# ZhonghuaYi/FocusFlow_official

Measured on AMD Instinct MI355X. Metric: frame-pairs/sec FF-RAFT 384x512 iters=12, higher is better.
Workload: dtype f32 via fp16x3 split operands on the f16 MFMA pipe (f32 accumulate, fp32-level accuracy); 1 GPU; FF-RAFT forward (test_mode), 8 pairs/GPU 384x512, iters=12, fp32 correlation pyramid, random-init weights, ORB-like masks (BASELINE configs[1]); pairs_per_gpu=8, corr_pyramid=fp32, conv_precision=f16x3, hipgraph=False, skip_unused_upsample=False, parallelism=dp1 (independent shards, no collective)

## Files before the change

### focusflow_official_amd/_hip.py

```python
import ctypes as C
import os

_PKG = os.path.dirname(os.path.abspath(__file__))
LIB_PATH = os.path.join(_PKG, "lib", "libfocusflow_hip.so")
if os.environ.get("FF_LAB_LIB"):
    LIB_PATH = os.path.join(_PKG, "lib", os.environ["FF_LAB_LIB"])

ACT_NONE, ACT_RELU, ACT_SIGMOID, ACT_TANH, ACT_LEAKY = 0, 1, 2, 3, 4
W_F32, W_F16X3, W_F16 = 0, 1, 2
MAX_SEG = 3
_fp = C.c_void_p
_ll = C.c_longlong


class FFFusionPair(C.Structure):
    _fields_ = [
        ("x", _fp * 2), ("x_ld", C.c_int * 2), ("xres", _fp * 2), ("xres_ld", C.c_int * 2), ("scale", _fp * 2), ("shift", _fp * 2),
        ("in_act", C.c_int), ("w_frag", _fp * 2), ("bias", _fp * 2), ("w_format", C.c_int), ("y", _fp * 2), ("y_ld", C.c_int * 2),
        ("B", C.c_int), ("HW", C.c_int), ("C", C.c_int),
    ]


class FFEncoderTail(C.Structure):
    _fields_ = [
        ("x", _fp * 2), ("x_ld", C.c_int * 2), ("xres", _fp * 2), ("xres_ld", C.c_int * 2), ("scale", _fp * 2), ("shift", _fp * 2),
        ("in_act", C.c_int), ("w_frag", _fp), ("bias", _fp), ("w_format", C.c_int), ("y", _fp), ("y_ld", C.c_int),
        ("B", C.c_int), ("HW", C.c_int), ("C", C.c_int), ("Cout", C.c_int),
    ]


class FFConvParams(C.Structure):
    _fields_ = [
        ("x", _fp * MAX_SEG), ("x_ld", C.c_int * MAX_SEG), ("x_c", C.c_int * MAX_SEG),
        ("x_gstride", _ll * MAX_SEG), ("groups", C.c_int), ("B", C.c_int), ("H", C.c_int), ("W", C.c_int),
        ("w", _fp), ("w_gstride", _ll), ("bias", _fp), ("ch_scale", _fp), ("ch_shift", _fp),
        ("out_scale", C.c_float), ("res", _fp), ("res_ld", C.c_int), ("y", _fp), ("y_ld", C.c_int),
        ("y_gstride", _ll), ("Ho", C.c_int), ("Wo", C.c_int), ("Cout", C.c_int),
        ("KH", C.c_int), ("KW", C.c_int), ("stride", C.c_int), ("pad_h", C.c_int), ("pad_w", C.c_int),
        ("act", C.c_int), ("act_res", C.c_int), ("w_format", C.c_int),
        ("dil_h", C.c_int), ("dil_w", C.c_int), ("x_amax", _fp),
        ("in_scale", _fp), ("in_shift", _fp), ("in_act", C.c_int),
        ("res2", _fp), ("res2_ld", C.c_int), ("res_split", C.c_int),
        ("splitk_ws", _fp), ("splitk", C.c_int),
        ("ep_mode", C.c_int), ("ep_split", C.c_int), ("ep_a", _fp), ("ep_a_ld", C.c_int), ("ep_b", _fp), ("ep_b_ld", C.c_int),
        ("stats_part", _fp),
        ("x_fmt", C.c_int * MAX_SEG), ("y_fmt", C.c_int), ("y_fmt_from", C.c_int), ("y2", _fp), ("y2_ld", C.c_int),
        ("w_frag", _fp),
    ]


PACK_MAX_MEMBERS = 4
PACK_MAX_SLICES = 4


class FFPackJob(C.Structure):
    _fields_ = [
        ("w", _fp * PACK_MAX_MEMBERS), ("bias", _fp * PACK_MAX_MEMBERS),
        ("cout_m", C.c_int * PACK_MAX_MEMBERS), ("off", C.c_int * PACK_MAX_MEMBERS), ("nmem", C.c_int), ("cout", C.c_int),
        ("cin_src", C.c_int), ("nslice", C.c_int), ("slice_lo", C.c_int * PACK_MAX_SLICES), ("slice_hi", C.c_int * PACK_MAX_SLICES),
        ("cin", C.c_int), ("cin_pad", C.c_int), ("KH", C.c_int), ("KW", C.c_int),
# ... 34 lines not shown
    "ff_corr_lookup_tiled_bwd_all": [_fp, C.POINTER(_fp), C.POINTER(_fp), C.c_int, C.c_int, _ll, C.c_int, C.c_int, _fp],
    "ff_corr_lookup_tiled_bwd": [C.POINTER(_fp), _fp, _fp, C.c_int, _ll, C.c_int, C.c_int, _fp],
    "ff_corr_pyramid_tiled_bwd": [_fp, _fp, _fp, _fp, _ll, C.c_int, C.c_int, _fp],
    "ff_corr_alt_prepare": [_fp, _fp, C.c_int, C.c_int, C.c_int, C.c_int, C.c_int, _fp, C.POINTER(_fp), _fp],
    "ff_corr_alt_lookup": [_fp, C.POINTER(_fp), C.c_int, _fp, C.c_int, C.c_int, C.c_int, _fp, C.c_int, _fp, _fp],
    "ff_corr_alt_lookup_bwd": [_fp, C.POINTER(_fp), C.POINTER(_fp), C.POINTER(_fp), C.c_int, C.c_int, C.c_int, C.c_int, C.c_int, _fp,
                               C.POINTER(_fp), _fp],
    "ff_act_copy": [_fp, C.c_int, _fp, C.c_int, _ll, C.c_int, C.c_int, _fp],
    "ff_range_probe": [_fp, C.c_int, _ll, C.c_int, _fp, _fp],
    "ff_split_copy": [_fp, C.c_int, _fp, C.c_int, _ll, C.c_int, C.c_int, C.c_int, _fp],
    "ff_coords_init": [_fp, _fp, C.c_int, C.c_int, C.c_int, _fp],
    "ff_forward_interpolate": [_fp, _fp, _fp, C.c_int, C.c_int, C.c_int, _fp],
    "ff_good_features": [_fp, C.c_int, _ll, _ll, _ll, C.c_int, C.c_int, C.c_int, C.c_int, C.c_double, C.c_int, _fp, _fp, _fp, _fp, _fp],
    "ff_frame_ingest": [_fp, _ll, _ll, _ll, _ll, C.c_int, C.c_int, C.c_int, C.c_int, C.c_int, C.c_int, C.c_int, C.c_int, _fp, _fp],
    "ff_pad_replicate": [_fp, C.c_int, _ll, _ll, _ll, C.c_int, C.c_int, C.c_int, C.c_int, C.c_int, C.c_int, C.c_int, _fp, _fp],
    "ff_keypoint_matches": [_fp, _fp, C.c_int, _fp, _ll, _ll, _ll, _ll, C.c_int, C.c_int, C.c_int, C.c_int, C.c_int, C.c_int, C.c_int, _fp, _fp, _fp],
    "ff_tracks_replenish": [_fp, _fp, _fp, _fp, C.c_int, _fp, _fp, C.c_int, C.c_int, C.c_int, C.c_int, C.c_int, _fp, _fp, _fp],
    "ff_tracks_mask": [_fp, _fp, C.c_int, C.c_int, C.c_int, C.c_int, _fp, _fp],
    "ff_tracks_advance": [_fp, _fp, _fp, C.c_int, _fp, _ll, _ll, _ll, _ll, C.c_int, C.c_int, C.c_int, C.c_int, C.c_int, C.c_int, C.c_int, _fp, _fp, _fp,
                          _fp, _fp],
    "ff_fb_dense": [_fp, _ll, _ll, _ll, _ll, _fp, _ll, _ll, _ll, _ll, C.c_int, C.c_int, C.c_int, C.c_int, C.c_int, C.c_int, C.c_int, C.c_float, C.c_float,
                    _fp, _fp, _fp],
    "ff_fb_matches": [_fp, _fp, C.c_int, _fp, _ll, _ll, _ll, _ll, C.c_int, C.c_int, C.c_int, C.c_int, C.c_int, C.c_int, C.c_int, C.c_float, C.c_float,
                      _fp, _fp, _fp, _fp, _fp, _fp],
    "ff_epipolar_ransac": [_fp, _fp, C.c_int, C.c_int, C.c_int, C.c_int, C.c_float, C.c_int, C.c_int, C.c_int, C.c_uint, _fp, C.c_int, _fp, _fp, _fp, _fp,
                           _fp, _fp, _fp, _fp, _fp, _fp, _ll, _fp],
    "ff_coords_step": [_fp, _fp, C.c_int, _fp, _fp, C.c_int, C.c_int, C.c_int, C.c_int, _fp],
    "ff_gru_pass": [C.c_int, _fp, C.c_int, _fp, C.c_int, _fp, C.c_int, _fp, C.c_int, _fp, C.c_int, _fp, _fp, _fp, _fp, C.c_int, _fp, C.c_int, _fp, C.c_int,
                    C.c_int, C.c_int, C.c_int, _fp],
    "ff_gru_pass_rec": [C.c_int, _fp, C.c_int, _fp, C.c_int, _fp, C.c_int, _fp, C.c_int, _fp, C.c_int, _fp, _fp, _fp, _fp, C.c_int, _fp, C.c_int, _fp, C.c_int,
                        _fp, _fp, _fp, C.c_int, C.c_int, C.c_int, C.c_int, _fp],
    "ff_fusion_pair_fwd": [C.POINTER(FFFusionPair), _fp],
    "ff_encoder_tail_fwd": [C.POINTER(FFEncoderTail), _fp],
    "ff_gru_rh": [_fp, C.c_int, _fp, C.c_int, _fp, C.c_int, _ll, C.c_int, _fp],
    "ff_gru_blend": [_fp, C.c_int, _fp, C.c_int, _fp, C.c_int, _fp, C.c_int, _ll, C.c_int, _fp],
    "ff_upsample_flow": [_fp, C.c_int, _fp, C.c_int, _fp, C.c_int, C.c_int, C.c_int, _fp],
    "ff_nhwc_to_nchw": [_fp, C.c_int, _fp, C.c_int, C.c_int, C.c_int, C.c_int, _fp],
    "ff_conv2d_wgrad": [C.POINTER(FFConvParams), _fp, _ll, _fp, _fp],
    "ff_unpack_conv_wgrad": [_fp, C.c_int, C.c_int, C.c_int, C.c_int, C.c_int, C.c_int, _fp, _fp],
    "ff_pack_conv_weight_dgrad": [_fp, C.c_int, C.c_int, C.c_int, C.c_int, _fp, C.c_int, C.c_int, _fp],
    "ff_act_bwd": [_fp, C.c_int, _fp, C.c_int, _fp, C.c_int, _ll, C.c_int, C.c_int, C.c_int, C.c_float, _fp, _fp],
    "ff_deconv4x4s2_small": [_fp, C.c_int, C.c_int, C.c_int, C.c_int, C.c_int, _fp, _fp, C.c_int, _fp, C.c_int, _fp],
    "ff_dilate2": [_fp, C.c_int, _fp, C.c_int, C.c_int, C.c_int, C.c_int, C.c_int, C.c_int, _fp],
    "ff_norm_bwd": [_fp, C.c_int, _fp, C.c_int, _fp, C.c_int, _fp, _fp, C.c_int, C.c_int, C.c_float, _fp, _fp,
                    C.c_int, _fp, C.c_int, _fp, C.c_int, C.c_int, C.c_int, C.c_int, _fp, _fp],
    "ff_gru_rh_bwd": [_fp, C.c_int, _fp, C.c_int, _fp, C.c_int, _fp, C.c_int, _fp, C.c_int, _ll, C.c_int, _fp],
    "ff_gru_blend_bwd": [_fp, C.c_int, _fp, C.c_int, _fp, C.c_int, _fp, C.c_int, _fp, C.c_int, _fp, C.c_int,
                         _fp, C.c_int, _ll, C.c_int, _fp],
    "ff_upsample_flow_bwd": [_fp, _fp, C.c_int, _fp, C.c_int, _fp, _fp, C.c_int, C.c_int, C.c_int, _fp],
    "ff_upsample_flow_bwd_ex": [_fp, _fp, C.c_int, _fp, C.c_int, _fp, C.c_int, _fp, C.c_float, _fp, C.c_int, C.c_int, C.c_int, _fp],
    "ff_gru_bwd_blend": [_fp, C.c_int, _fp, C.c_int, _fp, C.c_int, _fp, C.c_int, _fp, C.c_int, _fp, C.c_int, _fp, C.c_int, _fp, C.c_int, _fp, C.c_int,
                         _fp, _fp, _ll, C.c_int, _fp],
    "ff_gru_bwd_rh": [_fp, C.c_int, _fp, C.c_int, _fp, C.c_int, _fp, C.c_int, _fp, C.c_int, _fp, C.c_int, C.c_int, _fp, _ll, C.c_int, _fp],
    "ff_gru_bwd_out": [_fp, C.c_int, _fp, C.c_int, _fp, C.c_int, _fp, C.c_int, _fp, C.c_int, _fp, C.c_int, C.c_int, _fp, _ll, C.c_int, _fp],
    "ff_sum_stack": [_fp, C.c_int, _ll, _fp, _fp],
    "ff_pwc_costvolume_fwd": [_fp, C.c_int, _fp, C.c_int, _fp, C.c_int, C.c_int, C.c_int, C.c_int, C.c_int, _fp],
    "ff_pwc_costvolume_fwd_ex": [_fp, C.c_int, _fp, C.c_int, _fp, C.c_int, C.c_int, C.c_int, C.c_int, C.c_int, C.c_int, _fp, C.c_int, _fp],
    "ff_pwc_costvolume_bwd": [_fp, C.c_int, _fp, C.c_int, _fp, C.c_int, C.c_int, C.c_int, C.c_int, C.c_int, _fp],
    "ff_pwc_gout_transpose": [_fp, C.c_int, _fp, C.c_int, C.c_int, C.c_int, C.c_int, _fp],
    "ff_pwc_backwarp": [_fp, C.c_int, _fp, C.c_int, C.c_float, _fp, C.c_int, C.c_int, C.c_int, C.c_int, C.c_int, _fp],
    "ff_loss_prepare": [_fp, _fp, _fp, _fp, C.c_int, C.c_float, _fp, _fp, _fp, C.c_int, C.c_int, C.c_int, _fp],
    "ff_loss_accumulate": [_fp, _fp, _fp, _fp, _fp, C.c_float, C.c_float, C.c_float, _fp, _fp, C.c_int, C.c_int,
                           C.c_int, _fp],
    "ff_epe_metric": [_fp, _fp, _fp, _fp, C.c_int, C.c_int, C.c_int, _fp],
    "ff_nchw_to_nhwc4": [_fp, C.c_int, C.c_float, _fp, C.c_int, C.c_int, C.c_int, _fp],
    "ff_resize_bilinear": [_fp, C.c_int, C.c_int, C.c_int, C.c_int, _fp, C.c_int, C.c_int, C.c_int, C.c_float, C.c_float, _fp],
    "ff_pwc_backwarp_bwd": [_fp, C.c_int, _fp, C.c_int, C.c_float, _fp, C.c_int, _fp, C.c_int, _fp, C.c_int, C.c_int, C.c_int, C.c_int,
                            C.c_int, _fp],
    "ff_pwc_loss_mask": [_fp, _fp, C.c_int, _fp, _fp, C.c_int, C.c_int, C.c_int, C.c_int, C.c_int, _fp],
    "ff_pwc_loss_scale": [_fp, _fp, _fp, _fp, C.c_float, C.c_float, C.c_int, C.c_int, C.c_int, C.c_float, C.c_float, _fp, _fp, C.c_int,
                          C.c_int, C.c_int, C.c_int, C.c_int, _fp],
    "ff_pwc_epe_mean": [_fp, _fp, C.c_int, C.c_float, C.c_float, _fp, C.c_int, C.c_int, C.c_int, _fp],
    "ff_pwc_loss_scale_sparse": [_fp, _fp, _fp, _fp, C.c_float, C.c_float, C.c_int, C.c_int, C.c_int, C.c_float, C.c_float, _fp, _fp, C.c_int,
                                 C.c_int, C.c_int, C.c_int, C.c_int, _fp],
    "ff_pwc_epe_mean_sparse": [_fp, _fp, C.c_int, C.c_float, C.c_float, _fp, C.c_int, C.c_int, C.c_int, _fp],
    "ff_resize_to_nhwc4": [_fp, C.c_int, C.c_int, C.c_int, _fp, C.c_int, C.c_int, C.c_int, _fp],
    "ff_png_unfilter": [_fp, _ll, C.c_int, C.c_int, C.c_int, _fp],
    "ff_mask_prepare": [C.c_int, _fp, _fp, _fp, C.c_int, _fp, _fp, _fp, C.c_int, C.c_int, C.c_int, _fp],
    "ff_chan_stats_fwd": [_fp, C.c_int, C.c_int, _ll, _fp, C.c_int, _fp, _fp],
    "ff_chan_stats_bwd": [_fp, C.c_int, _fp, C.c_int, _ll, _fp, C.c_int, _fp],
    "ff_spatial_stats_fwd": [_fp, C.c_int, C.c_int, C.c_int, C.c_int, _fp, _fp, _fp, _fp, _fp],
    "ff_spatial_stats_bwd": [_fp, _fp, _fp, C.c_int, C.c_int, C.c_int, _fp, C.c_int, _fp],
    "ff_scale_add_fwd": [_fp, C.c_int, _fp, C.c_int, _fp, _fp, C.c_int, _fp, C.c_int, C.c_int, C.c_int, C.c_int, C.c_int, _fp],
    "ff_scale_add_bwd": [_fp, C.c_int, _fp, C.c_int, _fp, C.c_int, _fp, _fp, C.c_int, _fp, _fp, C.c_int, C.c_int, C.c_int,
                         C.c_int, _fp],
}
EXPORTS = sorted(list(_SIGS) + ["ff_last_error", "ff_abi_version", "ff_corr_plane_elems", "ff_conv2d_splitk_hint", "ff_conv2d_stats_parts", "ff_fusion_pair_tile",
                                 "ff_forward_interpolate_ws", "ff_good_features_ws", "ff_epipolar_ws"])

ABI_VERSION = 7
_lib = None


class FocusFlowHipError(RuntimeError):
    pass


_ABLATION_VARS = ("FF_LOOKUP_ABLATE", "FF_LOOKUP_ABLATE3", "FF_CORR_BUILD_ABLATE", "FF_PATCH_ABLATE")
_TUNING_VARS = ("FF_DMA_TILE", "FF_GRU_PASS_TH", "FF_LAB_LIB")


def lab_variables_set():
    return [v for v in _ABLATION_VARS + _TUNING_VARS if os.environ.get(v) is not None]


def load():
    global _lib
    if _lib is not None:
        return _lib
    abl = [v for v in _ABLATION_VARS if os.environ.get(v) is not None]
    if abl and not os.environ.get("FF_LAB_LIB"):
        raise FocusFlowHipError(f"{', '.join(abl)} set in the environment: timing-only ablations return wrong results and are not part of "
                                "libfocusflow_hip.so; unset them (the lab build under tools/ is where they live)")
    if not os.path.exists(LIB_PATH):
        raise FocusFlowHipError(
            f"{LIB_PATH} is missing: build it with `python -m focusflow_official_amd.build` "
            "(hipcc --offload-arch=gfx950).  There is no CPU/PyTorch fallback for the hot path.")
    lib = C.CDLL(LIB_PATH)
    for name, argtypes in _SIGS.items():
        fn = getattr(lib, name, None)
        if fn is None:
            raise FocusFlowHipError(f"{LIB_PATH} does not export {name}: it was built from older sources; "
                                    "rebuild with `python -m focusflow_official_amd.build`")
        fn.argtypes = argtypes
        fn.restype = C.c_int
    lib.ff_last_error.restype = C.c_char_p
    lib.ff_last_error.argtypes = []
    lib.ff_abi_version.restype = C.c_int
    lib.ff_abi_version.argtypes = []
    lib.ff_corr_plane_elems.restype = C.c_int
    lib.ff_corr_plane_elems.argtypes = [C.c_int, C.c_int, C.c_int, C.c_int]
    lib.ff_conv2d_splitk_hint.restype = C.c_int
    lib.ff_conv2d_splitk_hint.argtypes = [C.POINTER(FFConvParams)]
    lib.ff_fusion_pair_tile.restype = C.c_int
    lib.ff_fusion_pair_tile.argtypes = [C.c_int]
    lib.ff_forward_interpolate_ws.restype = C.c_int
    lib.ff_forward_interpolate_ws.argtypes = [C.c_int, C.c_int, C.c_int]
    lib.ff_good_features_ws.restype = C.c_int
    lib.ff_good_features_ws.argtypes = [C.c_int, C.c_int, C.c_int]
    lib.ff_epipolar_ws.restype = C.c_int
    lib.ff_epipolar_ws.argtypes = [C.c_int, C.c_int, C.c_int]
    lib.ff_conv2d_stats_parts.restype = C.c_int
    lib.ff_conv2d_stats_parts.argtypes = [C.POINTER(FFConvParams)]
    got = lib.ff_abi_version()
    if got != ABI_VERSION:
        raise FocusFlowHipError(f"{LIB_PATH} speaks ABI version {got}, these bindings (FFConvParams layout, argument lists) "
                                f"version {ABI_VERSION}: rebuild with `python -m focusflow_official_amd.build`")
    _lib = lib
    return lib


def call(name, *args):
    lib = load()
    rc = getattr(lib, name)(*args)
    if rc != 0:
        raise FocusFlowHipError(f"{name} failed ({rc}): {lib.ff_last_error().decode()}")
```

### focusflow_official_amd/cce.py

```python
from typing import Tuple, Optional, Sequence

import ctypes
import os
import weakref

import torch
import torch.nn as nn

from . import _hip, fn, ops
from .ops import ACT_NONE, ACT_RELU, ACT_SIGMOID

EPS = 1e-5


_NORM_ON_LOAD = True


_ALL_PACKED = weakref.WeakSet()
_DMA_FRAG = True
_PREPACK = True
_serial = [0]


class PackedConv:
# ... 275 lines not shown
            blk += (J.items_fwd + J.items_dgrad + 255) // 256
            arr[i] = J
        host = torch.frombuffer(bytearray(bytes(arr)), dtype=torch.uint8)
        cache = owner.__dict__["_ff_pack_table"] = (sig, host.to(device), len(jobs), blk)
    ops.pack_weights_table(cache[1], cache[2], cache[3])
    for (pc, nf, nd, kf, kd), (J, fmt, dfmt) in zip(todo, jobs):
        if nf:
            pc.w, pc.fmt, pc._key = (pc._w_raw if fmt == 0 else pc._w_split), fmt, kf
            pc._gen += 1
        if nd:
            pc.wd, pc.dfmt, pc._dkey = (pc._wd_raw if dfmt == 0 else pc._wd_split), dfmt, kd
    return len(todo)


def train_streams() -> bool:
    v = os.environ.get("FF_TRAIN_STREAMS")
    if v is not None:
        return v != "0"
    return not (torch.distributed.is_available() and torch.distributed.is_initialized())
_BRANCH_STREAMS = True
_branch_streams = {}


def _branch_stream(device):
    key = (torch.device(device).index, torch.cuda.current_stream(device).cuda_stream)
    if key not in _branch_streams:
        _branch_streams[key] = torch.cuda.Stream(device=device)
    return _branch_streams[key]


_FUSION_PAIR = os.environ.get("FF_FUSION_PAIR", "1") != "0"
_PAIR_FUSION = True
_ENCODER_TAIL = True
_W_LIMIT = 4094.0


def invalidate_packed(module: nn.Module) -> int:
    ids = {id(p) for p in module.parameters()}
    n = 0
    for pc in list(_ALL_PACKED):
        if id(pc.convs[0]._parameters["weight"]) in ids:
            pc._key = pc._dkey = None
            n += 1
    for m in module.modules():
        if hasattr(m, "_ff_fold"):
            del m._ff_fold
            n += 1
        if getattr(m, "_pair_key", None) is not None:
            m._pair_key = None
            n += 1
        if getattr(m, "_tail_key", None) is not None:
            m._tail_key = None
            n += 1
        if getattr(m, "_mask2_stage_of", None) is not None:
            m._mask2_stage = m._mask2_stage_of = None
            n += 1
    return n


def _make_norm(kind: str, c: int):
    if kind == "batch":
        return nn.BatchNorm2d(c)
    if kind == "instance":
        return nn.InstanceNorm2d(c)
    if kind == "none":
        return nn.Sequential()
# ... 167 lines not shown
                    return ops.LazyAct(y, st, y.shape[1] * y.shape[2], EPS, act, res)
                return ops.norm_apply(y, st, True, EPS, act=act, res=res, out=y)
            if ops.CONV_STATS_TRAIN:
                y, st = fn.conv(pc, x, want_stats=True, take_res=take_res)
            else:
                y = fn.conv(pc, x, take_res=take_res)
                st = ops.norm_stats(y.detach(), per_sample=True)
            return fn.NormFn.apply(y, None, None, res, True, False, EPS, relu, st, defer_res)
        if self.norm_fn == "batch":
            if norm.training:
                y = fn.conv(pc, x, take_res=take_res and taped)
                st = ops.norm_stats(y.detach(), per_sample=False)
                b, h, w, _ = y.shape
                ops.bn_update_running(norm, st, b * h * w)
                norm.num_batches_tracked += 1
                if taped:
                    return fn.NormFn.apply(y, norm.weight, norm.bias, res, False, False, norm.eps, relu, st, defer_res)
                return ops.norm_apply(y, st, False, norm.eps, norm.weight, norm.bias, act=act, res=res, out=y)
            if taped:
                y = fn.conv(pc, x, take_res=take_res)
                n = float(y.shape[0] * y.shape[1] * y.shape[2])
                rm, rv = norm.running_mean.double(), norm.running_var.double()
                st = torch.stack([rm * n, (rv + rm * rm) * n], -1)[None].contiguous()
                return fn.NormFn.apply(y, norm.weight, norm.bias, res, False, True, norm.eps, relu, st, defer_res)
            sc, sh = ops.bn_fold(norm)
            return pc(x, act=act, ch_scale=sc, ch_shift=sh, res=res, act_res=ACT_RELU)
        if taped:
            raise NotImplementedError("norm_fn='none' has no autograd path (unused by the reference configs)")
        return pc(x, act=act, res=res, act_res=ACT_RELU)

    def _block_recorded(self, blk: ResidualBlock, x) -> bool:
        return torch.is_grad_enabled() and x.requires_grad and self.norm_fn in ("instance", "batch")

    def _block(self, blk: ResidualBlock, x, lazy_out=False):
        p2 = blk._p2
        if (_NORM_ON_LOAD and self.norm_fn == "instance" and not torch.is_grad_enabled() and ops.w_format() in (_hip.W_F16X3, _hip.W_F16)
                and p2.cin % 32 == 0 and (p2.kh, p2.kw, p2.stride) == (3, 3, 1)):
            t1, st = blk._p1(x, want_stats=True)
            sc, sh = ops.norm_coeffs(st, t1.shape[1] * t1.shape[2], EPS)
            if blk.downsample is not None:
                x = self._conv_norm(x, blk._pd, blk.norm3, ACT_NONE)
            t2, st2 = p2(t1, in_scale=sc, in_shift=sh, in_act=ACT_RELU, want_stats=True)
            if lazy_out:
                return ops.LazyAct(t2, st2, t2.shape[1] * t2.shape[2], EPS, ACT_RELU, x)
            return ops.norm_apply(t2, st2, True, EPS, act=ACT_RELU, res=x, out=t2)
        fuse = blk.downsample is None and self._block_recorded(blk, x) and fn.res_grad_fused(blk._p1)
        y = self._conv_norm(x, blk._p1, blk.norm1, ACT_RELU, take_res=fuse)
        if blk.downsample is not None:
            x = self._conv_norm(x, blk._pd, blk.norm3, ACT_NONE)
        return self._conv_norm(y, blk._p2, blk.norm2, ACT_RELU, res=x, lazy=lazy_out and self.norm_fn == "instance" and not torch.is_grad_enabled(),
                               defer_res=fuse)

    def _run_stage(self, stage, x, lazy_out=False):
        if lazy_out:
            return self._block(stage[1], self._block(stage[0], x), True)
        return self._block(stage[1], self._block(stage[0], x))

    def _run_stem(self, x, lazy=False):
        return self._conv_norm(x, self._stem, self.norm1, ACT_RELU, lazy=lazy)

    def _run_out(self, x):
        return fn.conv(self._out, x)


class BasicEncoder(_ResidualEncoder):

    def __init__(self, in_channel=3, output_dim=128, norm_fn="batch", dropout=0.0):
        super().__init__()
        self.norm_fn = norm_fn
        if dropout and dropout > 0:
            raise NotImplementedError("dropout > 0 is not used by any reference config and is not built")
        if in_channel > 4:
            raise NotImplementedError(f"in_channel={in_channel}: the stem reads the NHWC4 images of ops.prep_input (at most 4 channels)")
        self._frame_layers(in_channel, output_dim)
        self.dropout = None
        self._init_weights()
        self._stem = PackedConv([self.conv1], 4)
        self._out = PackedConv([self.conv2])

    def forward(self, x, mask=None):
        x = self._run_stem(x)
        x = self._run_stage(self.layer1, x)
# ... 120 lines not shown
```

### focusflow_official_amd/ops.py

```python
import ctypes as C
import math
import os
import threading
from typing import List, Optional, Sequence

import torch

from . import _hip
from ._hip import ACT_LEAKY, ACT_NONE, ACT_RELU, ACT_SIGMOID, ACT_TANH, FFConvParams

Tensor = torch.Tensor


_raw_stream = getattr(torch._C, "_cuda_getCurrentRawStream", None)
_raw_device = getattr(torch._C, "_cuda_getDevice", None)


def _stream():
    if _raw_stream is not None and _raw_device is not None:
        return C.c_void_p(_raw_stream(_raw_device()))
    return C.c_void_p(torch.cuda.current_stream().cuda_stream)


_PRECISIONS = {"fp32": _hip.W_F32, "f16x3": _hip.W_F16X3, "f16": _hip.W_F16}
# ... 1240 lines not shown
    ins = (x, m)
    b, h, w, c = ins[0].shape
    p = _hip.FFEncoderTail()
    for i, v in enumerate(ins):
        t = v.t if isinstance(v, LazyAct) else v
        _require_gpu(t)
        if tuple(t.shape[:3]) != (b, h, w):
            raise _hip.FocusFlowHipError(f"encoder_tail: inputs of different shapes {tuple(ins[0].shape)} / {tuple(t.shape)}")
        c = min(c, t.shape[3])
        p.x[i], p.x_ld[i] = t.data_ptr(), _ld(t)
        if isinstance(v, LazyAct):
            sc, sh = v.coeffs()
            p.scale[i], p.shift[i] = sc.data_ptr(), sh.data_ptr()
            p.in_act = v.act
            if v.res is not None:
                p.xres[i], p.xres_ld[i] = v.res.data_ptr(), _ld(v.res)
    acts = {v.act for v in ins if isinstance(v, LazyAct)}
    assert len(acts) <= 1, "lazy inputs of one stage share the activation"
    if _range_word is not None:
        for v in ins:
            probe = v.res if isinstance(v, LazyAct) else v
            if probe is not None:
                _range_probe(probe)
    _require_gpu(bias)
    cout = bias.numel()
    y = empty_nhwc(b, h, w, cout, bias)
    p.w_frag, p.bias, p.w_format = w_frag.data_ptr(), bias.data_ptr(), w_fmt
    p.y, p.y_ld = y.data_ptr(), cout
    p.B, p.HW, p.C, p.Cout = b, h * w, c, cout
    _timed_call("conv", "ff_encoder_tail_fwd", C.byref(p), _stream(), note=(2.0 * b * h * w * 2 * c * cout, w_fmt))
    return y


def mask_upsample_pack(w_split: Tensor) -> Tensor:
    assert w_split.dtype == torch.uint8 and w_split.numel() == 576 * 1024 and w_split.is_contiguous()
    out = torch.empty_like(w_split)
    _hip.call("ff_mask_upsample_pack", _p(w_split), _p(out), _stream())
    return out


def mask_upsample(hid: Tensor, w_stage: Tensor, w_fmt: int, bias: Optional[Tensor], flow: Tensor, out_scale: float = 0.25) -> Tensor:
    b, h, w, c = hid.shape
    assert c == 256 and w_fmt in (_hip.W_F16X3, _hip.W_F16) and flow.shape[:3] == (b, h, w)
    out = torch.empty((b, 2, 8 * h, 8 * w), dtype=torch.float32, device=hid.device)
    _hip.call("ff_mask_upsample_fwd", _p(hid), _ld(hid), _p(w_stage), w_fmt, _p(bias), out_scale, _p(flow), _ld(flow), _p(out), b, h, w, _stream())
    return out


def upsample_flow(flow: Tensor, mask: Tensor) -> Tensor:
    b, h, w, _ = flow.shape
    out = torch.empty((b, 2, 8 * h, 8 * w), dtype=torch.float32, device=flow.device)
    _hip.call("ff_upsample_flow", _p(flow), _ld(flow), _p(mask), _ld(mask), _p(out), b, h, w, _stream())
    return out


def nhwc_to_nchw(x: Tensor) -> Tensor:
    b, h, w, c = x.shape
    out = torch.empty((b, c, h, w), dtype=torch.float32, device=x.device)
    _hip.call("ff_nhwc_to_nchw", _p(x), _ld(x), _p(out), b, h, w, c, _stream())
    return out


def _conv_params(xs, b, h, w, cout, kh, kw, stride, pad, ho, wo, dilation=1):
    p = FFConvParams()
    p.dil_h = p.dil_w = dilation
    for i, x in enumerate(xs):
# ... 251 lines not shown
```

### include/focusflow_hip.h

```cpp
#ifndef FOCUSFLOW_HIP_H
#define FOCUSFLOW_HIP_H

#ifdef __cplusplus
extern "C" {
#endif

#define FF_OK 0
#define FF_EINVAL (-1)
#define FF_EHIP (-2)

#define FF_ACT_NONE 0
#define FF_ACT_RELU 1
#define FF_ACT_SIGMOID 2
#define FF_ACT_TANH 3
#define FF_ACT_LEAKY 4

#define FF_MAX_SEG 3

#define FF_W_F32 0
#define FF_W_F16X3 1
#define FF_W_F16 2

const char* ff_last_error(void);
#define FF_ABI_VERSION 7
// ... 164 lines not shown
int ff_gru_pass(int dir, const float* hs, int hs_ld, const float* motion, int mo_ld, const float* h, int h_ld,
                const float* zr_pre, int zr_pre_ld, const float* q_pre, int q_pre_ld, const void* wzr_frag, const void* wq_frag,
                const float* bzr, const float* bq, int w_format, float* y, int y_ld, float* y2, int y2_ld, int B, int H, int W,
                void* stream);
int ff_gru_pass_rec(int dir, const float* hs, int hs_ld, const float* motion, int mo_ld, const float* h, int h_ld,
                    const float* zr_pre, int zr_pre_ld, const float* q_pre, int q_pre_ld, const void* wzr_frag, const void* wq_frag,
                    const float* bzr, const float* bq, int w_format, float* y, int y_ld, float* y2, int y2_ld, float* z, float* r,
                    float* q, int gate_ld, int B, int H, int W, void* stream);
typedef struct FFFusionPair {
    const float* x[2];     int x_ld[2];
    const float* xres[2];  int xres_ld[2];
    const float* scale[2]; const float* shift[2];
    int in_act;
    const void* w_frag[2];
    const float* bias[2];
    int w_format;
    float* y[2];           int y_ld[2];
    int B, HW, C;
} FFFusionPair;
int ff_fusion_pair_tile(int C);
int ff_fusion_pair_fwd(const FFFusionPair* p, void* stream);
typedef struct FFEncoderTail {
    const float* x[2];     int x_ld[2];
    const float* xres[2];  int xres_ld[2];
    const float* scale[2]; const float* shift[2];
    int in_act;
    const void* w_frag;
    const float* bias;
    int w_format;
    float* y;              int y_ld;
    int B, HW, C, Cout;
} FFEncoderTail;
int ff_encoder_tail_fwd(const FFEncoderTail* p, void* stream);
int ff_gru_rh(const float* r, int r_ld, const float* h, int h_ld, float* rh, int rh_ld,
              long long npix, int C, void* stream);
int ff_gru_blend(const float* z, int z_ld, const float* q, int q_ld, const float* h, int h_ld,
                 float* h_new, int hn_ld, long long npix, int C, void* stream);
int ff_mask_upsample_pack(const void* w_split, void* w_stage, void* stream);
int ff_mask_upsample_fwd(const float* hid, int hid_ld, const void* w_stage, int w_format, const float* bias, float out_scale,
                         const float* flow, int flow_ld, float* out, int B, int H, int W, void* stream);
int ff_upsample_flow(const float* flow, int flow_ld, const float* mask, int mask_ld,
                     float* out_nchw, int B, int H, int W, void* stream);
int ff_nhwc_to_nchw(const float* src, int ld, float* dst, int B, int H, int W, int C, void* stream);

int ff_conv2d_wgrad(const FFConvParams* p, float* dw, long long dw_gstride, float* db, void* stream);
int ff_unpack_conv_wgrad(const float* packed, int Cout, int Cin, int KH, int KW, int cin_pad,
                         int cout_offset, float* dw_oihw, void* stream);
int ff_pack_conv_weight_dgrad(const float* w_oihw, int Cout, int Cin, int KH, int KW, float* dst,
                              int cout_pad, int cout_offset, void* stream);
#define FF_PACK_MAX_MEMBERS 4
#define FF_PACK_MAX_SLICES 4
typedef struct FFPackJob {
    const float* w[FF_PACK_MAX_MEMBERS];
    const float* bias[FF_PACK_MAX_MEMBERS];
    int cout_m[FF_PACK_MAX_MEMBERS], off[FF_PACK_MAX_MEMBERS];
    int nmem, cout;
    int cin_src;
    int nslice, slice_lo[FF_PACK_MAX_SLICES], slice_hi[FF_PACK_MAX_SLICES];
    int cin, cin_pad, KH, KW;
    void* fwd;
    float* bias_dst;
    void* dgrad;
    int fwd_format, dgrad_format, cout_pad, reserved;
    long long items_fwd;
    long long items_dgrad;
    long long block0;
// ... 99 lines not shown
```

Measured before the change: 633.8 frame-pairs/s.

## Fuse stride-2 3x3 conv and 1x1 downsample shortcut into one kernel

Adds a HIP kernel that computes a residual block's 3x3 stride-2 conv and its 1x1 stride-2 downsample shortcut together. It stages the shared input tile once in LDS, split into fp16 terms, and runs both on MFMA. The center tap of the 3x3 reuses the same LDS data for the 1x1. Bias, folded batchnorm and ReLU, or per-tile instance-norm statistics, are applied in the epilogue. This removes one full read of the input and one kernel launch per downsampling block in the encoders, at the cost of a specialised kernel with fixed tile shape and a Cout of only 96 or 128.

```diff
diff --git a/focusflow_official_amd/_hip.py b/focusflow_official_amd/_hip.py
--- a/focusflow_official_amd/_hip.py
+++ b/focusflow_official_amd/_hip.py
@@ -26,6 +26,15 @@
         ("x", _fp * 2), ("x_ld", C.c_int * 2), ("xres", _fp * 2), ("xres_ld", C.c_int * 2), ("scale", _fp * 2), ("shift", _fp * 2),
         ("in_act", C.c_int), ("w_frag", _fp), ("bias", _fp), ("w_format", C.c_int), ("y", _fp), ("y_ld", C.c_int),
         ("B", C.c_int), ("HW", C.c_int), ("C", C.c_int), ("Cout", C.c_int),
+    ]
+
+
+class FFConvS2Pair(C.Structure):
+    _fields_ = [
+        ("x", _fp), ("x_ld", C.c_int), ("B", C.c_int), ("H", C.c_int), ("W", C.c_int), ("Cin", C.c_int), ("Cout", C.c_int),
+        ("k", C.c_int * 2), ("stride", C.c_int * 2), ("pad", C.c_int * 2), ("w3_frag", _fp), ("w1_frag", _fp), ("w_format", C.c_int),
+        ("bias", _fp * 2), ("scale", _fp * 2), ("shift", _fp * 2), ("act", C.c_int * 2), ("y", _fp * 2), ("y_ld", C.c_int * 2),
+        ("stats_part", _fp * 2),
     ]
 
 
@@ -126,6 +135,7 @@
                         _fp, _fp, _fp, C.c_int, C.c_int, C.c_int, C.c_int, _fp],
     "ff_fusion_pair_fwd": [C.POINTER(FFFusionPair), _fp],
     "ff_encoder_tail_fwd": [C.POINTER(FFEncoderTail), _fp],
+    "ff_conv_s2_pair_fwd": [C.POINTER(FFConvS2Pair), _fp],
     "ff_gru_rh": [_fp, C.c_int, _fp, C.c_int, _fp, C.c_int, _ll, C.c_int, _fp],
     "ff_gru_blend": [_fp, C.c_int, _fp, C.c_int, _fp, C.c_int, _fp, C.c_int, _ll, C.c_int, _fp],
     "ff_upsample_flow": [_fp, C.c_int, _fp, C.c_int, _fp, C.c_int, C.c_int, C.c_int, _fp],
@@ -180,7 +190,7 @@
                          C.c_int, _fp],
 }
 EXPORTS = sorted(list(_SIGS) + ["ff_last_error", "ff_abi_version", "ff_corr_plane_elems", "ff_conv2d_splitk_hint", "ff_conv2d_stats_parts", "ff_fusion_pair_tile",
-                                 "ff_forward_interpolate_ws", "ff_good_features_ws", "ff_epipolar_ws"])
+                                 "ff_forward_interpolate_ws", "ff_good_features_ws", "ff_epipolar_ws", "ff_conv_s2_pair_stats_parts"])
 
 ABI_VERSION = 7
 _lib = None
@@ -236,6 +246,8 @@
     lib.ff_epipolar_ws.argtypes = [C.c_int, C.c_int, C.c_int]
     lib.ff_conv2d_stats_parts.restype = C.c_int
     lib.ff_conv2d_stats_parts.argtypes = [C.POINTER(FFConvParams)]
+    lib.ff_conv_s2_pair_stats_parts.restype = C.c_int
+    lib.ff_conv_s2_pair_stats_parts.argtypes = [C.c_int, C.c_int]
     got = lib.ff_abi_version()
     if got != ABI_VERSION:
         raise FocusFlowHipError(f"{LIB_PATH} speaks ABI version {got}, these bindings (FFConvParams layout, argument lists) "
diff --git a/focusflow_official_amd/cce.py b/focusflow_official_amd/cce.py
--- a/focusflow_official_amd/cce.py
+++ b/focusflow_official_amd/cce.py
@@ -331,6 +331,7 @@
 _FUSION_PAIR = os.environ.get("FF_FUSION_PAIR", "1") != "0"
 _PAIR_FUSION = True
 _ENCODER_TAIL = True
+_S2_PAIR = True
 _W_LIMIT = 4094.0
 
 
@@ -564,22 +565,56 @@
     def _block_recorded(self, blk: ResidualBlock, x) -> bool:
         return torch.is_grad_enabled() and x.requires_grad and self.norm_fn in ("instance", "batch")
 
+    def _s2_pair(self, blk: ResidualBlock, x):
+        p1, pd = blk._p1, blk._pd
+        if not (_S2_PAIR and pd is not None and not torch.is_grad_enabled() and ops.w_format() in (_hip.W_F16X3, _hip.W_F16)):
+            return None
+        if self.norm_fn == "batch":
+            if blk.norm1.training or blk.norm3.training:
+                return None
+        elif self.norm_fn != "instance":
+            return None
+        geom = lambda pc: (pc.kh, pc.kw, pc.stride, pc.pad, pc.dil)
+        if (geom(p1) != (3, 3, 2, (1, 1), 1) or geom(pd) != (1, 1, 2, (0, 0), 1) or (p1.cin, p1.cout) != (pd.cin, pd.cout)
+                or p1.cin_pad != p1.cin or pd.cin_pad != pd.cin or p1.force_f32 or pd.force_f32 or not p1.plain or not pd.plain
+                or not ops.conv_s2_pair_inputs_ok(x, p1.cout) or x.shape[3] != p1.cin):
+            return None
+        (_, b3), (_, b1) = p1.get(), pd.get()
+        w3, w1 = p1.frag(), pd.frag()
+        if self.norm_fn == "instance":
+            return ops.conv_s2_pair(x, w3, w1, b3, b1, p1.cout, p1.fmt, want_stats=True)
+        (s3, h3), (s1, h1) = ops.bn_fold(blk.norm1), ops.bn_fold(blk.norm3)
+        return ops.conv_s2_pair(x, w3, w1, b3, b1, p1.cout, p1.fmt, scale=(s3, s1), shift=(h3, h1), act=(ACT_RELU, ACT_NONE))
+
     def _block(self, blk: ResidualBlock, x, lazy_out=False):
         p2 = blk._p2
+        pair = self._s2_pair(blk, x) if blk.downsample is not None else None
         if (_NORM_ON_LOAD and self.norm_fn == "instance" and not torch.is_grad_enabled() and ops.w_format() in (_hip.W_F16X3, _hip.W_F16)
                 and p2.cin % 32 == 0 and (p2.kh, p2.kw, p2.stride) == (3, 3, 1)):
-            t1, st = blk._p1(x, want_stats=True)
+            if pair is not None:
+                t1, st, d, std = pair
+            else:
+                t1, st = blk._p1(x, want_stats=True)
             sc, sh = ops.norm_coeffs(st, t1.shape[1] * t1.shape[2], EPS)
-            if blk.downsample is not None:
+            if pair is not None:
+                x = ops.norm_apply(d, std, True, EPS, act=ACT_NONE, out=d)
+            elif blk.downsample is not None:
                 x = self._conv_norm(x, blk._pd, blk.norm3, ACT_NONE)
             t2, st2 = p2(t1, in_scale=sc, in_shift=sh, in_act=ACT_RELU, want_stats=True)
             if lazy_out:
                 return ops.LazyAct(t2, st2, t2.shape[1] * t2.shape[2], EPS, ACT_RELU, x)
             return ops.norm_apply(t2, st2, True, EPS, act=ACT_RELU, res=x, out=t2)
         fuse = blk.downsample is None and self._block_recorded(blk, x) and fn.res_grad_fused(blk._p1)
-        y = self._conv_norm(x, blk._p1, blk.norm1, ACT_RELU, take_res=fuse)
-        if blk.downsample is not None:
-            x = self._conv_norm(x, blk._pd, blk.norm3, ACT_NONE)
+        if pair is not None and self.norm_fn == "instance":
+            t1, st, d, std = pair
+            y = ops.norm_apply(t1, st, True, EPS, act=ACT_RELU, out=t1)
+            x = ops.norm_apply(d, std, True, EPS, act=ACT_NONE, out=d)
+        elif pair is not None:
+            y, x = pair
+        else:
+            y = self._conv_norm(x, blk._p1, blk.norm1, ACT_RELU, take_res=fuse)
+            if blk.downsample is not None:
+                x = self._conv_norm(x, blk._pd, blk.norm3, ACT_NONE)
         return self._conv_norm(y, blk._p2, blk.norm2, ACT_RELU, res=x, lazy=lazy_out and self.norm_fn == "instance" and not torch.is_grad_enabled(),
                                defer_res=fuse)
 
diff --git a/focusflow_official_amd/csrc/conv_s2_pair.hip b/focusflow_official_amd/csrc/conv_s2_pair.hip
--- /dev/null
+++ b/focusflow_official_amd/csrc/conv_s2_pair.hip
@@ -0,0 +1,236 @@
+#include <algorithm>
+#include "ff_common.h"
+
+namespace {
+
+typedef float f32x4 __attribute__((ext_vector_type(4)));
+typedef _Float16 f16x8 __attribute__((ext_vector_type(8)));
+typedef unsigned u32x4 __attribute__((__vector_size__(4 * sizeof(unsigned))));
+
+__device__ __forceinline__ int PI16(int i) { return (i >= 4 && i < 12) ? 2 * (i - 4) : (i < 4 ? 2 * i + 1 : 2 * (i - 12) + 9); }
+__device__ __forceinline__ int slot_of(int g) { return ((g & 1) << 1) | (g >> 1); }
+
+constexpr int TH = 4, TW = 16;
+constexpr int PH = 2 * TH + 1, PW = 2 * TW + 1;
+constexpr int NEV = TW + 1;
+constexpr int NPOS = PH * PW;
+constexpr int PITCH = 144;
+constexpr int LDS_BYTES = NPOS * PITCH;
+constexpr unsigned OOB = 0x80000000u;
+
+struct SArgs {
+    FFConvS2Pair p;
+    int Ho, Wo, tiles_x, tiles_y, ncin;
+    unsigned x_bytes, y_bytes[2];
+};
+
+template <int TERMS, int NW>
+__global__ __launch_bounds__(NW * 64) __attribute__((amdgpu_waves_per_eu(NW == 8 ? 4 : 5, NW == 8 ? 4 : 5))) void conv_s2_pair_kernel(const SArgs a) {
+    constexpr int NT = NW * 64, NITEM = NPOS * 8, NJ = (NITEM + NT - 1) / NT;
+    __shared__ __attribute__((aligned(16))) char smem[LDS_BYTES];
+    const FFConvS2Pair& p = a.p;
+    const int tid = threadIdx.x, lane = tid & 63, wave = tid >> 6;
+    const int i16 = lane & 15, g16 = lane >> 4;
+    const int tx = blockIdx.x, ty = blockIdx.y, b = blockIdx.z;
+    const int ox0 = tx * TW, oy0 = ty * TH, ix0 = 2 * ox0 - 1, iy0 = 2 * oy0 - 1;
+    const int H = p.H, W = p.W, ncin = a.ncin;
+
+    const __amdgpu_buffer_rsrc_t rx = __builtin_amdgcn_make_buffer_rsrc(const_cast<float*>(p.x), 0, a.x_bytes, 0x00020000);
+
+    unsigned goff[NJ];
+    int loff[NJ];
+#pragma unroll
+    for (int j = 0; j < NJ; ++j) {
+        const int i = tid + j * NT, pos = i >> 3, q = i & 7;
+        const int r = pos / PW, c = pos - r * PW;
+        const int iy = iy0 + r, ix = ix0 + c;
+        const bool ok = i < NITEM && (unsigned)iy < (unsigned)H && (unsigned)ix < (unsigned)W;
+        goff[j] = ok ? ((unsigned)((b * H + iy) * W + ix) * (unsigned)p.x_ld) * 4u + q * 16 : OOB;
+        const int idx = (c & 1) ? NEV + (c >> 1) : (c >> 1);
+        loff[j] = (r * PW + idx) * PITCH + slot_of(q >> 1) * 16 + (q & 1) * 8;
+    }
+
+    const __amdgpu_buffer_rsrc_t rwa = __builtin_amdgcn_make_buffer_rsrc(const_cast<void*>(p.w3_frag), 0, NW * 9 * ncin * 2048, 0x00020000);
+    const __amdgpu_buffer_rsrc_t rwd = __builtin_amdgcn_make_buffer_rsrc(const_cast<void*>(p.w1_frag), 0, NW * ncin * 2048, 0x00020000);
+    const int wbase_a = lane * 16 + wave * 9 * ncin * 2048, wbase_d = lane * 16 + wave * ncin * 2048;
+
+    f32x4 acc_a[TH], acc_d[TH];
+#pragma unroll
+    for (int py = 0; py < TH; ++py) acc_a[py] = acc_d[py] = (f32x4){0.f, 0.f, 0.f, 0.f};
+    const int pxl = PI16(i16);
+    const char* bp = smem + pxl * PITCH + slot_of(g16) * 16;
+
+    auto load_w = [&](const __amdgpu_buffer_rsrc_t r, int off, f32x4 (&wv)[2]) {
+        wv[0] = __builtin_bit_cast(f32x4, __builtin_amdgcn_raw_buffer_load_b128(r, off, 0, 0));
+        if (TERMS == 3) wv[1] = __builtin_bit_cast(f32x4, __builtin_amdgcn_raw_buffer_load_b128(r, off + 1024, 0, 0));
+    };
+    auto tap_step = [&](const char* xp, const f32x4 (&wv)[2], f32x4 (&acc)[TH]) {
+        const f16x8 w0 = __builtin_bit_cast(f16x8, wv[0]);
+        f16x8 w1;
+        if (TERMS == 3) w1 = __builtin_bit_cast(f16x8, wv[1]);
+#pragma unroll
+        for (int py = 0; py < TH; ++py) {
+            const f16x8 xa = *reinterpret_cast<const f16x8*>(xp + py * (2 * PW * PITCH));
+            acc[py] = __builtin_amdgcn_mfma_f32_16x16x32_f16(w0, xa, acc[py], 0, 0, 0);
+            if (TERMS == 3) {
+                const f16x8 xb = *reinterpret_cast<const f16x8*>(xp + py * (2 * PW * PITCH) + 64);
+                acc[py] = __builtin_amdgcn_mfma_f32_16x16x32_f16(w1, xa, acc[py], 0, 0, 0);
+                acc[py] = __builtin_amdgcn_mfma_f32_16x16x32_f16(w0, xb, acc[py], 0, 0, 0);
+            }
+            if (py == 1) __builtin_amdgcn_sched_barrier(0);
+        }
+    };
+    auto tap_off = [](int s) {
+        const int ky = (s * 11) >> 5, kx = s - 3 * ky;
+        return (ky * PW + (kx == 0 ? 0 : (kx == 1 ? NEV : 1))) * PITCH;
+    };
+
+    for (int kc = 0; kc < ncin; ++kc) {
+        f32x4 wc[2], wn[2];
+        {
+            f32x4 val[NJ];
+#pragma unroll
+            for (int j = 0; j < NJ; ++j) val[j] = __builtin_bit_cast(f32x4, __builtin_amdgcn_raw_buffer_load_b128(rx, goff[j] + kc * 128, 0, 0));
+            load_w(rwa, wbase_a + kc * 2048, wc);
+            if (kc) __syncthreads();
+#pragma unroll
+            for (int j = 0; j < NJ; ++j) {
+                if (j == NJ - 1 && tid + j * NT >= NITEM) continue;
+                ff::ff_f16x4 h0, h1;
+                ff::split_pair4(val[j], h0, h1);
+                *reinterpret_cast<ff::ff_f16x4*>(smem + loff[j]) = h0;
+                if (TERMS == 3) *reinterpret_cast<ff::ff_f16x4*>(smem + loff[j] + 64) = h1;
+            }
+        }
+        __syncthreads();
+#pragma unroll 1
+        for (int s = 0; s < 8; ++s) {
+            load_w(rwa, wbase_a + ((s + 1) * ncin + kc) * 2048, wn);
+            tap_step(bp + tap_off(s), wc, acc_a);
+            wc[0] = wn[0];
+            wc[1] = wn[1];
+        }
+        load_w(rwd, wbase_d + kc * 2048, wn);
+        tap_step(bp + tap_off(8), wc, acc_a);
+        tap_step(bp + tap_off(4), wn, acc_d);
+    }
+
+    const int Cout = NW * 16, ch = wave * 16 + g16 * 4;
+    const int ox = ox0 + pxl;
+    const int nparts = a.tiles_x * a.tiles_y, part = ty * a.tiles_x + tx;
+#pragma unroll
+    for (int o = 0; o < 2; ++o) {
+        const __amdgpu_buffer_rsrc_t ry = __builtin_amdgcn_make_buffer_rsrc(p.y[o], 0, a.y_bytes[o], 0x00020000);
+        const f32x4 bias = p.bias[o] ? *reinterpret_cast<const f32x4*>(p.bias[o] + ch) : (f32x4){0.f, 0.f, 0.f, 0.f};
+        f32x4 cs = {1.f, 1.f, 1.f, 1.f}, ct = {0.f, 0.f, 0.f, 0.f};
+        if (p.scale[o]) {
+            cs = *reinterpret_cast<const f32x4*>(p.scale[o] + ch);
+            ct = *reinterpret_cast<const f32x4*>(p.shift[o] + ch);
+        }
+        f32x4 out[TH];
+        bool ok[TH];
+#pragma unroll
+        for (int py = 0; py < TH; ++py) {
+            f32x4 v = (o == 0 ? acc_a[py] : acc_d[py]) * ff::SPLIT_INV + bias;
+            if (p.scale[o]) v = v * cs + ct;
+            if (p.act[o] == FF_ACT_RELU) {
+#pragma unroll
+                for (int r = 0; r < 4; ++r) v[r] = v[r] < 0.f ? 0.f : v[r];
+            }
+            out[py] = v;
+            const int oy = oy0 + py;
+            ok[py] = oy < a.Ho && ox < a.Wo;
+            const unsigned yoff = ok[py] ? ((unsigned)((b * a.Ho + oy) * a.Wo + ox) * (unsigned)p.y_ld[o] + ch) * 4u : OOB;
+            __builtin_amdgcn_raw_buffer_store_b128(__builtin_bit_cast(u32x4, v), ry, yoff, 0, 0);
+        }
+        if (p.stats_part[o]) {
+            f32x4* e = reinterpret_cast<f32x4*>(p.stats_part[o]) + ((long long)b * nparts + part) * Cout + ch;
+#pragma unroll
+            for (int r = 0; r < 4; ++r) {
+                float st_p = 0.f, st_s1 = 0.f, st_s2 = 0.f, st_n = 0.f;
+#pragma unroll
+                for (int py = 0; py < TH; ++py) {
+                    if (!ok[py]) continue;
+                    if (st_n == 0.f) st_p = out[py][r];
+                    const float d = out[py][r] - st_p;
+                    st_s1 += d;
+                    st_s2 = fmaf(d, d, st_s2);
+                    st_n += 1.f;
+                }
+#pragma unroll
+                for (int m = 1; m < 16; m <<= 1) {
+                    const float p2 = __shfl_xor(st_p, m), s2 = __shfl_xor(st_s1, m), q2 = __shfl_xor(st_s2, m), n2 = __shfl_xor(st_n, m);
+                    const float pv = st_n > 0.f ? st_p : p2, d = p2 - pv;
+                    st_s1 = st_s1 + s2 + n2 * d;
+                    st_s2 = st_s2 + q2 + 2.f * d * s2 + n2 * d * d;
+                    st_n += n2;
+                    st_p = pv;
+                }
+                if (i16 == 0) e[r] = (f32x4){st_p, st_s1, st_s2, st_n};
+            }
+        }
+    }
+}
+
+bool overlap(const void* a, long long na, const void* b, long long nb) {
+    const char *x = static_cast<const char*>(a), *y = static_cast<const char*>(b);
+    return x < y + nb && y < x + na;
+}
+
+template <int TERMS>
+void launch(const SArgs& a, hipStream_t s) {
+    const dim3 grid(a.tiles_x, a.tiles_y, a.p.B);
+    if (a.p.Cout == 96) conv_s2_pair_kernel<TERMS, 6><<<grid, 384, 0, s>>>(a);
+    else conv_s2_pair_kernel<TERMS, 8><<<grid, 512, 0, s>>>(a);
+}
+
+}
+
+extern "C" int ff_conv_s2_pair_stats_parts(int H, int W) {
+    if (H <= 0 || W <= 0) return 0;
+    const int Ho = (H - 1) / 2 + 1, Wo = (W - 1) / 2 + 1;
+    return ((Ho + TH - 1) / TH) * ((Wo + TW - 1) / TW);
+}
+
+extern "C" int ff_conv_s2_pair_fwd(const FFConvS2Pair* pp, void* stream) {
+    FF_REQUIRE(pp, "ff_conv_s2_pair_fwd: null argument");
+    const FFConvS2Pair& p = *pp;
+    FF_REQUIRE(p.k[0] == 3 && p.stride[0] == 2 && p.pad[0] == 1 && p.k[1] == 1 && p.stride[1] == 2 && p.pad[1] == 0,
+               "ff_conv_s2_pair_fwd: kernel / stride / pad (%d, %d, %d) + (%d, %d, %d): this entry runs a 3x3 stride-2 pad-1 convolution with a 1x1 stride-2 pad-0 shortcut",
+               p.k[0], p.stride[0], p.pad[0], p.k[1], p.stride[1], p.pad[1]);
+    FF_REQUIRE(p.w_format == FF_W_F16X3 || p.w_format == FF_W_F16, "ff_conv_s2_pair_fwd: w_format %d (a split weight format; fp32 rows take ff_conv2d_fwd)", p.w_format);
+    FF_REQUIRE(p.B > 0 && p.B < 65536 && p.H > 0 && p.W > 0, "ff_conv_s2_pair_fwd: B %d, H %d, W %d", p.B, p.H, p.W);
+    FF_REQUIRE(p.Cin > 0 && p.Cin % 32 == 0, "ff_conv_s2_pair_fwd: Cin = %d (a multiple of 32)", p.Cin);
+    FF_REQUIRE(p.Cout == 96 || p.Cout == 128, "ff_conv_s2_pair_fwd: Cout = %d (96 or 128; other widths take ff_conv2d_fwd)", p.Cout);
+    FF_REQUIRE(p.x && p.w3_frag && p.w1_frag && ff::aligned16(p.w3_frag) && ff::aligned16(p.w1_frag), "ff_conv_s2_pair_fwd: null input / weights, or weights not 16-byte aligned");
+    FF_REQUIRE(p.x_ld >= p.Cin && p.x_ld % 4 == 0 && ff::aligned16(p.x), "ff_conv_s2_pair_fwd: input: leading dimension %d (>= Cin, a multiple of 4) / 16-byte alignment", p.x_ld);
+    SArgs a;
+    a.p = p;
+    a.Ho = (p.H - 1) / 2 + 1;
+    a.Wo = (p.W - 1) / 2 + 1;
+    a.tiles_x = (a.Wo + TW - 1) / TW;
+    a.tiles_y = (a.Ho + TH - 1) / TH;
+    a.ncin = p.Cin / 32;
+    FF_REQUIRE(a.tiles_y < 65536, "ff_conv_s2_pair_fwd: H %d", p.H);
+    const long long xb = (((long long)p.B * p.H * p.W - 1) * p.x_ld + p.Cin) * 4;
+    FF_REQUIRE(xb < (1ll << 31), "ff_conv_s2_pair_fwd: a tensor of 2 GiB or more");
+    a.x_bytes = (unsigned)xb;
+    long long yb[2];
+    for (int o = 0; o < 2; ++o) {
+        FF_REQUIRE(p.y[o] && p.y_ld[o] >= p.Cout && p.y_ld[o] % 4 == 0 && ff::aligned16(p.y[o]),
+                   "ff_conv_s2_pair_fwd: output %d: null, leading dimension %d (>= Cout, a multiple of 4) or not 16-byte aligned", o, p.y_ld[o]);
+        yb[o] = (((long long)p.B * a.Ho * a.Wo - 1) * p.y_ld[o] + p.Cout) * 4;
+        FF_REQUIRE(yb[o] < (1ll << 31), "ff_conv_s2_pair_fwd: a tensor of 2 GiB or more");
+        a.y_bytes[o] = (unsigned)yb[o];
+        FF_REQUIRE(!overlap(p.y[o], yb[o], p.x, xb), "ff_conv_s2_pair_fwd: output %d aliases the input", o);
+        FF_REQUIRE(p.act[o] == FF_ACT_NONE || p.act[o] == FF_ACT_RELU, "ff_conv_s2_pair_fwd: act %d (FF_ACT_NONE or FF_ACT_RELU)", p.act[o]);
+        FF_REQUIRE(!p.bias[o] || ff::aligned16(p.bias[o]), "ff_conv_s2_pair_fwd: bias %d not 16-byte aligned", o);
+        FF_REQUIRE(!p.scale[o] || (p.shift[o] && ff::aligned16(p.scale[o]) && ff::aligned16(p.shift[o])), "ff_conv_s2_pair_fwd: scale without shift / alignment (output %d)", o);
+        FF_REQUIRE(!p.stats_part[o] || ff::aligned16(p.stats_part[o]), "ff_conv_s2_pair_fwd: stats_part %d not 16-byte aligned", o);
+    }
+    FF_REQUIRE(!overlap(p.y[0], yb[0], p.y[1], yb[1]), "ff_conv_s2_pair_fwd: the two outputs alias");
+    hipStream_t s = static_cast<hipStream_t>(stream);
+    if (p.w_format == FF_W_F16X3) launch<3>(a, s);
+    else launch<1>(a, s);
+    return ff::check_launch("ff_conv_s2_pair_fwd");
+}
diff --git a/focusflow_official_amd/ops.py b/focusflow_official_amd/ops.py
--- a/focusflow_official_amd/ops.py
+++ b/focusflow_official_amd/ops.py
@@ -1296,6 +1296,61 @@
     return y
 
 
+def conv_s2_pair_stats_parts(h: int, w: int) -> int:
+    return _hip.load().ff_conv_s2_pair_stats_parts(h, w)
+
+
+def conv_s2_pair_inputs_ok(x, cout: int) -> bool:
+    if not isinstance(x, Tensor) or x.dim() != 4 or not x.is_cuda or x.dtype != torch.float32:
+        return False
+    b, h, w, c = x.shape
+    if c % 32 or cout not in (96, 128) or x.stride(3) != 1 or x.data_ptr() % 16 or b >= 65536:
+        return False
+    ld = x.stride(2) if w > 1 else (x.stride(1) if h > 1 else max(x.stride(0), c))
+    if ld % 4 or ld < c or (w > 1 and h > 1 and x.stride(1) != w * ld) or (b > 1 and x.stride(0) != h * w * ld):
+        return False
+    return b * h * w * ld * 4 < (1 << 31)
+
+
+def conv_s2_pair(x: Tensor, w3_frag: Tensor, w1_frag: Tensor, bias3: Optional[Tensor], bias1: Optional[Tensor], cout: int, w_fmt: int,
+                 scale=(None, None), shift=(None, None), act=(ACT_NONE, ACT_NONE), want_stats: bool = False, out=(None, None),
+                 kernels=((3, 2, 1), (1, 2, 0))):
+    _require_gpu(x)
+    b, h, w, cin = x.shape
+    ho, wo = (h - 1) // 2 + 1, (w - 1) // 2 + 1
+    p = _hip.FFConvS2Pair()
+    p.x, p.x_ld = x.data_ptr(), _ld(x)
+    p.B, p.H, p.W, p.Cin, p.Cout = b, h, w, cin, cout
+    for i, (k, s, pd) in enumerate(kernels):
+        p.k[i], p.stride[i], p.pad[i] = k, s, pd
+    p.w3_frag, p.w1_frag, p.w_format = w3_frag.data_ptr(), w1_frag.data_ptr(), w_fmt
+    outs, parts = [], []
+    nparts = conv_s2_pair_stats_parts(h, w) if want_stats else 0
+    for i, bias in enumerate((bias3, bias1)):
+        y = out[i] if out[i] is not None else empty_nhwc(b, ho, wo, cout, x)
+        assert tuple(y.shape) == (b, ho, wo, cout)
+        outs.append(y)
+        p.y[i], p.y_ld[i] = y.data_ptr(), _ld(y)
+        p.bias[i] = bias.data_ptr() if bias is not None else None
+        if scale[i] is not None:
+            p.scale[i], p.shift[i] = scale[i].data_ptr(), shift[i].data_ptr()
+        p.act[i] = act[i]
+        if nparts:
+            parts.append(torch.empty(b * nparts * cout * 4, dtype=torch.float32, device=x.device))
+            p.stats_part[i] = parts[i].data_ptr()
+    if _range_word is not None:
+        _range_probe(x)
+    _timed_call("conv", "ff_conv_s2_pair_fwd", C.byref(p), _stream(), note=(2.0 * b * ho * wo * cout * cin * 10, w_fmt))
+    if not want_stats:
+        return outs[0], outs[1]
+    stats = []
+    for i in range(2):
+        st = _zero_stats(b, cout, x.device)
+        _hip.call("ff_norm_stats_finish", _p(parts[i]), b, nparts, cout, _p(st), _stream())
+        stats.append(st)
+    return outs[0], stats[0], outs[1], stats[1]
+
+
 def mask_upsample_pack(w_split: Tensor) -> Tensor:
     assert w_split.dtype == torch.uint8 and w_split.numel() == 576 * 1024 and w_split.is_contiguous()
     out = torch.empty_like(w_split)
diff --git a/include/focusflow_hip.h b/include/focusflow_hip.h
--- a/include/focusflow_hip.h
+++ b/include/focusflow_hip.h
@@ -220,6 +220,19 @@
     int B, HW, C, Cout;
 } FFEncoderTail;
 int ff_encoder_tail_fwd(const FFEncoderTail* p, void* stream);
+typedef struct FFConvS2Pair {
+    const float* x;        int x_ld;
+    int B, H, W, Cin, Cout;
+    int k[2], stride[2], pad[2];
+    const void* w3_frag;   const void* w1_frag;
+    int w_format;
+    const float* bias[2];  const float* scale[2]; const float* shift[2];
+    int act[2];
+    float* y[2];           int y_ld[2];
+    float* stats_part[2];
+} FFConvS2Pair;
+int ff_conv_s2_pair_stats_parts(int H, int W);
+int ff_conv_s2_pair_fwd(const FFConvS2Pair* p, void* stream);
 int ff_gru_rh(const float* r, int r_ld, const float* h, int h_ld, float* rh, int rh_ld,
               long long npix, int C, void* stream);
 int ff_gru_blend(const float* z, int z_ld, const float* q, int q_ld, const float* h, int h_ld,
```

Measured after the change: 640.6 frame-pairs/s (median of 6 runs). 1.1% higher.
